# imulki/serenade

Measured on AMD Instinct MI355X. Metric: mel frames/sec converted (UNet ODE + vocoder), 80x1024, higher is better.
Workload: dtype f32

## Files before the change

### include/serenade_hip.h

```cpp
#ifndef SERENADE_HIP_H
#define SERENADE_HIP_H

#include <stdint.h>

#ifdef __cplusplus
extern "C" {
#endif

#define SRN_ABI_VERSION 4
#define SRN_MAX_TAPS 16

enum { SRN_ACT_NONE = 0, SRN_ACT_LEAKY = 1, SRN_ACT_SILU = 2, SRN_ACT_MISH = 3 };
enum { SRN_RES_NONE = 0, SRN_RES_ADD = 1, SRN_RES_AXPY = 2 };
enum {
  SRN_POST_NONE = 0,
  SRN_POST_DIV = 1,
  SRN_POST_TANH = 2,
  SRN_POST_RELU = 3,
  SRN_POST_LEAKY = 4,
  SRN_POST_GELU = 5
};
enum {
  SRN_PREC_FP32 = 0,
  SRN_PREC_BF16X3 = 1,
  SRN_PREC_BF16X6 = 2
};
enum {
  SRN_ROUTE_AUTO = 0,
  SRN_ROUTE_TILED = 1,
  SRN_ROUTE_HALO = 2,
  SRN_ROUTE_GENERIC = 3,
  SRN_ROUTE_STRIP = 4,
  SRN_ROUTE_FAST_FP32 = 5
};
enum {
  SRN_FAMILY_GENERIC = 0,
  SRN_FAMILY_F32 = 1,
  SRN_FAMILY_FAST = 2,
  SRN_FAMILY_HALO = 3,
  SRN_FAMILY_STRIP = 4
};

typedef struct SrnConvParams {
  int32_t n_batch;
  int32_t n_head;
  int32_t T_in, T_out;
  int32_t C_in;
  int32_t C_in0;
  int32_t C_w;
  int32_t N;
  int32_t N_out;
  int32_t n_taps;
  int32_t tap_off[SRN_MAX_TAPS];
  int32_t in_stride;
  int32_t pad_reflect;
  int32_t w_nmajor;
  int32_t pro_act;
  float pro_slope;
  float alpha;
  float beta;
  int32_t geglu;
  int32_t res_mode;
  int32_t post;
  float post_div;
  int32_t out_t_stride, out_t_off;
  int32_t tile;
  const float* in0; int64_t in0_bs, in0_hs; int32_t ld_in0;
  const float* in1; int64_t in1_bs; int32_t ld_in1;
  const float* w;   int64_t w_bs, w_hs; int32_t ldw;
  const float* bias;
  const int32_t* len_in;
  const int32_t* len_out;
  const float* res;  int64_t res_bs, res_hs; int32_t ld_res;
  const float* res2; int64_t res2_bs; int32_t ld_res2;
  float* out; int64_t out_bs, out_hs; int32_t ld_out;
  int32_t precision;
  int32_t route;
  void* ws; int64_t ws_bytes;
  const void* w_hi; const void* w_lo;
  float* gn_partials;
  float* out_tr; int64_t out_tr_bs; int32_t ld_out_tr; int32_t out_tr_col0;
} SrnConvParams;

int srn_abi_version(void);
const char* srn_last_error(void);

int srn_conv_gemm(const SrnConvParams* p, void* stream);
int64_t srn_conv_gemm_workspace_bytes(const SrnConvParams* p);
int srn_conv_gemm_route(const SrnConvParams* p, int32_t out[3]);

int srn_gn_mish_apply(const float* x, const float* gn_partials, const float* gamma, const float* beta,
                      const float* time_bias, int64_t time_bias_bs, const int32_t* lens, float* y, int B, int T,
                      int C, int groups, float eps, int valid_stats, void* stream);

int srn_resblock_tail(const float* c2, const float* gn_partials, const float* gamma, const float* beta,
                      const int32_t* lens, const float* r, const float* scale, const float* shift, int64_t ld_ss,
                      float* y, int B, int T, int C, int groups, float gn_eps, float ln_eps, int valid_stats,
                      void* stream);

int srn_resblock_tail_ln(const float* c2, const float* gn_partials, const float* gamma, const float* beta,
                         const int32_t* lens, const float* r, const float* scale, const float* shift, int64_t ld_ss,
                         float* y, int B, int T, int C, int groups, float gn_eps, float ln_eps, int valid_stats,
                         const float* ln2_gamma, const float* ln2_beta, float* y2, float ln2_eps, void* stream);

int srn_layernorm(const float* x, const float* gamma, const float* beta, float* y, int64_t rows, int C, float eps,
                  void* stream);

int srn_softmax_rows(float* s, const int32_t* lens, int Z, int n_head, int L, int ld, void* stream);

int srn_sinusoidal_emb(const float* t, float* out, int n, int dim, int ld, float scale, void* stream);

int srn_copy_channels(const float* src, int64_t src_bs, int ld_src, int sc0, float* dst, int64_t dst_bs, int ld_dst,
                      int dc0, int B, int T, int C, void* stream);

int srn_scatter_rows(const float* src, int64_t src_bs, int ld_src, float* dst, int64_t dst_bs, int ld_dst, int dc0,
                     const int32_t* row_off, const int32_t* n_rows, int B, int T, int C, void* stream);

int srn_transpose_ct(const float* src, float* dst, int B, int R, int Cc, int64_t src_bs, int ld_src, int64_t dst_bs,
                     int ld_dst, void* stream);
#define SRN_TR_LIST_MAX 40
typedef struct SrnTransposeList {
  int32_t n;
  int32_t pad_;
  const float* src[SRN_TR_LIST_MAX];
  float* dst[SRN_TR_LIST_MAX];
  int64_t src_bs[SRN_TR_LIST_MAX], dst_bs[SRN_TR_LIST_MAX];
  int32_t B[SRN_TR_LIST_MAX], R[SRN_TR_LIST_MAX], Cc[SRN_TR_LIST_MAX];
  int32_t ld_src[SRN_TR_LIST_MAX], ld_dst[SRN_TR_LIST_MAX];
  int32_t first_block[SRN_TR_LIST_MAX + 1];
} SrnTransposeList;
int srn_transpose_multi(const SrnTransposeList* list, void* stream);

int srn_renorm(const float* x, const float* trg_scale, const float* trg_mean, const float* voc_mean,
               const float* voc_scale, float* y, int64_t rows, int C, void* stream);

int srn_out_conv_tanh(const float* x, const float* w, const float* bias, float* y, int B, int T, int C, int k,
                      float slope, void* stream);

typedef struct SrnResUnitParams {
  int32_t n_batch, T, C;
  int32_t k, dilation;
  float slope;
  const float* x; int64_t x_bs;
  const float* w1; const float* b1; const float* w2; const float* b2;
  const void* w1_hi; const void* w2_hi;
  const float* res2; int64_t res2_bs;
  float post_div;
  float* out; int64_t out_bs;
  int32_t precision;
  int32_t route;
} SrnResUnitParams;
enum { SRN_RESUNIT_ROUTE_SHARED = 1 };

int srn_hifigan_resunit(const SrnResUnitParams* p, void* stream);

int srn_pd_gather(const float* x, const float* d, float* out, int B, int T, int C, float dilation, float slope,
                  void* stream);

int srn_gru_recur_last(const float* gi, const float* w_hh_t, const float* b_hh, float* h, int B, int T, int H,
                       void* stream);

int srn_style_token_attention_kv(const float* ref, const float* wq_t, const float* bq, const float* k, const float* v,
                                 const float* wo_t, const float* bo, float* out, int B, int Dq, int n_tok, int F,
                                 int n_head, void* stream);

int srn_pad_signal(const float* x, float* out, int B, int n, int pad, int ld, int mode, void* stream);
int srn_logmel(const float* spec, const float* mel_t, float* out, int64_t frames, int n_bins, int ld, int n_mels,
               float eps, int log_mode, void* stream);
int srn_loudness(const float* spec, const float* a_weight_db, uint32_t* gmax_ws, float* out, int B, int frames,
                 int n_bins, int ld, float amin, float top_db, float add_eps, void* stream);

int srn_rowln_fwd(const float* x, const float* m, int64_t m_bs, const float* a, int64_t a_bs, float* y, int B, int T,
                  int C, float eps, void* stream);
int srn_rowln_bwd(const float* x, const float* dy, const float* m, int64_t m_bs, float* dx, float* partial, int B, int T,
                  int C, float eps, void* stream);
int srn_rowln_chunks(int T);
int srn_gn_mish_bwd_partial(const float* h, const float* dy, const float* mean, const float* rstd, const float* gamma,
                            const float* beta, const int32_t* lens, float* partial, int B, int T, int C, int groups,
                            void* stream);
int srn_gn_mish_bwd_apply(const float* h, const float* dy, const float* mean, const float* rstd, const float* gamma,
                          const float* beta, const float* gsum, const int32_t* lens, float* dh, int B, int T, int C,
                          int groups, void* stream);
int srn_gn_chunks(int T);
int srn_gn_stats(const float* partials, float* mean, float* rstd, int B, int T, int C, int groups, float eps,
                 void* stream);
int srn_chunk_colsum(const float* partial, const float* gamma, float* col, float* gsum, int B, int n_chunk, int C,
                     int groups, void* stream);
int srn_colsum(const float* x, float* partial, float* out, int B, int64_t R, int N, int ld, void* stream);
int srn_colsum_chunks(int64_t R);
int srn_softmax_bwd(const float* p, float* dp, int64_t rows, int L, int ld, float scale, void* stream);
int srn_geglu_fwd(const float* hg, float* a, int64_t rows, int inner, void* stream);
int srn_geglu_bwd(const float* hg, const float* da, float* dhg, int64_t rows, int inner, void* stream);
int srn_adamw(float* p, const float* g, float* m, float* v, int64_t n, float lr, float beta1, float beta2, float eps,
              float weight_decay, int step, float grad_scale, void* stream);
int srn_adamw_dyn(float* p, const float* g, float* m, float* v, int64_t n, float beta1, float beta2, float eps,
                  float weight_decay, const float* dyn, void* stream);
int srn_sumsq(const float* g, int64_t n, double* partial, void* stream);
int srn_dot(const float* a, const float* b, int64_t n, double* partial, void* stream);
#define SRN_COPY_LIST_MAX 160
typedef struct SrnCopyList {
  int32_t n;
  int32_t pad_;
  const void* src[SRN_COPY_LIST_MAX];
  int64_t off[SRN_COPY_LIST_MAX];
  int64_t len[SRN_COPY_LIST_MAX];
} SrnCopyList;
int srn_multi_copy(const SrnCopyList* list, float* dst, void* stream);
int srn_sumsq_blocks(int64_t n);
int srn_weight_norm_fwd(const float* v, const float* g, float* w_packed, float* wd, float* inv_norm, int N, int C, int k,
                        void* stream);
int srn_weight_norm_bwd(const float* dw_packed, const float* v, const float* g, const float* inv_norm, float* dv,
                        float* dg, int N, int C, int k, void* stream);

typedef struct SrnWorldParams {
  int32_t n_batch, max_frames;
  int32_t fs, fft_size;
  const double* x; int64_t x_bs; const int32_t* x_len;
  const double* f0; const double* t; int64_t f_bs;
  const int32_t* n_frames;
  const double* twiddle;
  double q1, f0_floor;
  double threshold;
  double unvoiced_db;
  const double* band_window; int32_t band_window_len;
  int32_t n_bands;
  double* out0; int64_t out0_bs; int32_t ld_out0;
  double* out1; int64_t out1_bs; int32_t ld_out1;
} SrnWorldParams;
int srn_world_cheaptrick(const SrnWorldParams* p, void* stream);
int srn_world_d4c(const SrnWorldParams* p, void* stream);
int srn_world_project(const double* in, int64_t rows, int K, int ld_in, const double* mat_t, int n_out, int take_log,
                      double* out, int ld_out, void* stream);
int srn_world_pack_features(const double* a, int na, const double* b, int nb, const double* mean, const double* scale,
                            float* out, int64_t rows, int ld_out, void* stream);
int srn_wave_to_f64(const float* wave, double* out, int64_t n, int pcm16, void* stream);
int srn_f0_match_length(const double* in, int64_t in_bs, const int32_t* n_in, double* out, int64_t out_bs,
                        const int32_t* n_out, int n_batch, int max_out, void* stream);
int srn_cont_f0(const double* f0, int64_t bs, const int32_t* n_frames, double* cf0, float* uv, int32_t* ok,
                int n_batch, void* stream);
typedef struct SrnExcitationParams {
  int32_t n_batch, max_frames, fs, hop;
  const double* f0;
  const double* df_f0;
  int64_t f_bs;
  const int32_t* n_frames;
  double* phase_ws;
  const float* noise;
  float* sine;
  float sine_amp, noise_amp;
  int32_t n_df;
  float* dfs[4];
  int32_t df_upsample[4];
  double dense_factors[4];
} SrnExcitationParams;
int srn_sifigan_excitation(const SrnExcitationParams* p, void* stream);

typedef struct SrnTnGemmParams {
  int32_t n_batch, n_head;
  int32_t n_items, T_a, T_b;
  int32_t stride, n_shifts;
  int32_t shift[SRN_MAX_TAPS];
  int32_t M, N;
  const float* a; int64_t a_bs, a_hs, a_is; int32_t lda;
  const float* b; int64_t b_bs, b_hs, b_is; int32_t ldb;
  float* out; int64_t out_bs, out_hs; int32_t ldc;
  float alpha;
  float* ws; int64_t ws_bytes;
  int32_t n_inner;
  int64_t a_is2, b_is2;
  const int32_t* len_b;
  float* colsum;
  int32_t route;
} SrnTnGemmParams;
enum { SRN_TN_ROUTE_GENERAL = 1 };
int srn_tn_gemm(const SrnTnGemmParams* p, void* stream);
int64_t srn_tn_gemm_workspace_bytes(const SrnTnGemmParams* p);

int srn_bn_chunks(int64_t rows);
int srn_bn_relu_fwd(const float* x, const float* gamma, const float* beta, float* run_mean, float* run_var,
                    float* partial, float* stats, float* y, int64_t rows, int C, float eps, float momentum, void* stream);
int srn_bn_relu_bwd(const float* x, const float* y, const float* dy, const float* stats, const float* gamma,
                    float* partial, float* sums, float* dx, int64_t rows, int C, void* stream);
int srn_im2col_s2(const float* x, float* col, int B, int H, int W, int C, int ld, void* stream);
int srn_col2im_s2(const float* col, float* dx, int B, int H, int W, int C, int ld, void* stream);
int srn_gru_train_fwd(const float* gi, const float* w_hh_t, const float* b_hh, float* hs, float* gates, int B, int T,
                      int H, void* stream);
int srn_gru_train_bwd(const float* dh_last, const float* w_hh, const float* hs, const float* gates, float* dgi,
                      float* dgh, int B, int T, int H, void* stream);
int srn_token_attn_fwd(const float* q, const float* k, const float* v, float* p, float* ctx, int B, int n_tok, int F,
                       int n_head, void* stream);
int srn_token_attn_bwd(const float* dctx, const float* q, const float* k, const float* v, const float* p, float* dq,
                       float* dk_part, float* dv_part, int B, int n_tok, int F, int n_head, void* stream);

int srn_frame_stats_chunks(int T);
int srn_cvec_conv0(const float* wave, int64_t wave_bs, int n, const int32_t* lens, const float* w, float* out,
                   double* partials, int B, int T0, int C, int k, int stride, void* stream);
int srn_channel_norm_gelu(const float* x, const double* partials, int n_chunks, const int32_t* lens,
                          const float* gamma, const float* beta, float* stats, float* y, int B, int T, int C, float eps,
                          void* stream);
int srn_posconv_gelu_res(const float* x, const int32_t* lens, const float* w, const float* bias, float* y, int B,
                         int T, int C, int groups, int k, int pad, void* stream);

int srn_pad_ragged(const float* x, int64_t x_bs, const int32_t* lens, float* out, int B, int n, int pad, int ld,
                   void* stream);
int srn_mel_db(const float* spec, int ld_spec, int n_bins, const float* mel_t, const int32_t* lens, unsigned* gmax_ws,
               float* out, int ld_out, int B, int T, int n_mels, float amin, float top_db, void* stream);
int srn_trans_conv0(const float* x, int64_t x_bs, int ld_x, const int32_t* lens, const float* w, const float* bias,
                    float* out, int B, int T, int F, int C, int dilation, void* stream);
int srn_trans_pool(const float* in, const int32_t* lens, float* out, int B, int T, int F_in, int C, int C_valid,
                   int flatten, int ld_out, void* stream);
int srn_bilstm_slices(int H);
int srn_bilstm_recur(const float* g, int64_t g_bs, int ld_g, const int32_t* lens, const float* w_hh_t, float* out,
                     int64_t out_bs, int ld_out, int B, int T, int H, void* stream);

#define SRN_PYIN_MAX_FRAME 4096
#define SRN_PYIN_MAX_PERIODS 1024
#define SRN_PYIN_MAX_STATES 4096
#define SRN_PYIN_MAX_THRESHOLDS 1024
int srn_pyin_observe(const float* x, int64_t x_bs, const int32_t* lens, const int32_t* frames, const double* thresholds,
                     const double* beta_probs, const double* boltz_fact, const double* boltz_exp,
                     const double* no_trough, double* obs, double* voiced_prob, int B, int N, int T, int frame_length,
                     int win_length, int hop_length, int pad, int min_period, int max_period, int n_thresholds,
                     double sr, double fmin, double bins_per_octave, int n_bins, void* stream);
int srn_pyin_viterbi(const double* obs, const double* voiced_prob, const int32_t* frames, const double* log_band,
                     const double* log_p_init, const double* freqs, double log_tiny, double fill_na, int fill_unvoiced,
                     uint16_t* ptr_ws, int32_t* states, double* f0, uint8_t* voiced_flag, int B, int T, int n_bins,
                     int width, void* stream);

#ifdef __cplusplus
}
#endif
#endif
```

### serenade_amd/_lib.py

```python
import ctypes
import os
from ctypes import POINTER, c_char_p, c_double, c_float, c_int, c_int32, c_int64, c_void_p

_HERE = os.path.dirname(os.path.abspath(__file__))
LIB_PATH = os.environ.get("SERENADE_AMD_LIB") or os.path.join(_HERE, "libserenade_hip.so")

SRN_MAX_TAPS = 16
ACT_NONE, ACT_LEAKY, ACT_SILU, ACT_MISH = 0, 1, 2, 3
RES_NONE, RES_ADD, RES_AXPY = 0, 1, 2
POST_NONE, POST_DIV, POST_TANH, POST_RELU, POST_LEAKY, POST_GELU = 0, 1, 2, 3, 4, 5
PREC_FP32, PREC_BF16X3, PREC_BF16X6 = 0, 1, 2
ROUTE_AUTO, ROUTE_TILED, ROUTE_HALO, ROUTE_GENERIC, ROUTE_STRIP, ROUTE_FAST_FP32 = 0, 1, 2, 3, 4, 5
FAMILY_GENERIC, FAMILY_F32, FAMILY_FAST, FAMILY_HALO, FAMILY_STRIP = 0, 1, 2, 3, 4
RESUNIT_ROUTE_SHARED = 1
TN_ROUTE_GENERAL = 1


class SrnConvParams(ctypes.Structure):
    _fields_ = [
        ("n_batch", c_int32), ("n_head", c_int32), ("T_in", c_int32), ("T_out", c_int32),
        ("C_in", c_int32), ("C_in0", c_int32), ("C_w", c_int32), ("N", c_int32), ("N_out", c_int32),
        ("n_taps", c_int32), ("tap_off", c_int32 * SRN_MAX_TAPS), ("in_stride", c_int32),
        ("pad_reflect", c_int32), ("w_nmajor", c_int32), ("pro_act", c_int32), ("pro_slope", c_float),
        ("alpha", c_float), ("beta", c_float), ("geglu", c_int32), ("res_mode", c_int32), ("post", c_int32), ("post_div", c_float),
        ("out_t_stride", c_int32), ("out_t_off", c_int32), ("tile", c_int32),
        ("in0", c_void_p), ("in0_bs", c_int64), ("in0_hs", c_int64), ("ld_in0", c_int32),
        ("in1", c_void_p), ("in1_bs", c_int64), ("ld_in1", c_int32),
        ("w", c_void_p), ("w_bs", c_int64), ("w_hs", c_int64), ("ldw", c_int32),
        ("bias", c_void_p), ("len_in", c_void_p), ("len_out", c_void_p),
        ("res", c_void_p), ("res_bs", c_int64), ("res_hs", c_int64), ("ld_res", c_int32),
        ("res2", c_void_p), ("res2_bs", c_int64), ("ld_res2", c_int32),
        ("out", c_void_p), ("out_bs", c_int64), ("out_hs", c_int64), ("ld_out", c_int32),
        ("precision", c_int32), ("route", c_int32), ("ws", c_void_p), ("ws_bytes", c_int64),
        ("w_hi", c_void_p), ("w_lo", c_void_p), ("gn_partials", c_void_p),
        ("out_tr", c_void_p), ("out_tr_bs", c_int64), ("ld_out_tr", c_int32), ("out_tr_col0", c_int32),
    ]


class SrnResUnitParams(ctypes.Structure):
    _fields_ = [
        ("n_batch", c_int32), ("T", c_int32), ("C", c_int32), ("k", c_int32), ("dilation", c_int32),
        ("slope", c_float), ("x", c_void_p), ("x_bs", c_int64),
        ("w1", c_void_p), ("b1", c_void_p), ("w2", c_void_p), ("b2", c_void_p),
        ("w1_hi", c_void_p), ("w2_hi", c_void_p), ("res2", c_void_p), ("res2_bs", c_int64),
        ("post_div", c_float), ("out", c_void_p), ("out_bs", c_int64), ("precision", c_int32), ("route", c_int32),
    ]


SRN_COPY_LIST_MAX = 160


class SrnCopyList(ctypes.Structure):
    _fields_ = [("n", c_int32), ("pad_", c_int32), ("src", c_void_p * SRN_COPY_LIST_MAX),
                ("off", c_int64 * SRN_COPY_LIST_MAX), ("len", c_int64 * SRN_COPY_LIST_MAX)]


class SrnWorldParams(ctypes.Structure):
    _fields_ = [
        ("n_batch", c_int32), ("max_frames", c_int32), ("fs", c_int32), ("fft_size", c_int32),
        ("x", c_void_p), ("x_bs", c_int64), ("x_len", c_void_p),
        ("f0", c_void_p), ("t", c_void_p), ("f_bs", c_int64), ("n_frames", c_void_p), ("twiddle", c_void_p),
        ("q1", c_double), ("f0_floor", c_double), ("threshold", c_double), ("unvoiced_db", c_double),
        ("band_window", c_void_p), ("band_window_len", c_int32), ("n_bands", c_int32),
        ("out0", c_void_p), ("out0_bs", c_int64), ("ld_out0", c_int32),
        ("out1", c_void_p), ("out1_bs", c_int64), ("ld_out1", c_int32),
    ]


SRN_TR_LIST_MAX = 40


class SrnTransposeList(ctypes.Structure):
    _fields_ = [("n", c_int32), ("pad_", c_int32), ("src", c_void_p * SRN_TR_LIST_MAX), ("dst", c_void_p * SRN_TR_LIST_MAX),
                ("src_bs", c_int64 * SRN_TR_LIST_MAX), ("dst_bs", c_int64 * SRN_TR_LIST_MAX),
                ("B", c_int32 * SRN_TR_LIST_MAX), ("R", c_int32 * SRN_TR_LIST_MAX), ("Cc", c_int32 * SRN_TR_LIST_MAX),
                ("ld_src", c_int32 * SRN_TR_LIST_MAX), ("ld_dst", c_int32 * SRN_TR_LIST_MAX),
                ("first_block", c_int32 * (SRN_TR_LIST_MAX + 1))]


class SrnTnGemmParams(ctypes.Structure):
    _fields_ = [
        ("n_batch", c_int32), ("n_head", c_int32), ("n_items", c_int32), ("T_a", c_int32), ("T_b", c_int32),
        ("stride", c_int32), ("n_shifts", c_int32), ("shift", c_int32 * SRN_MAX_TAPS), ("M", c_int32), ("N", c_int32),
        ("a", c_void_p), ("a_bs", c_int64), ("a_hs", c_int64), ("a_is", c_int64), ("lda", c_int32),
        ("b", c_void_p), ("b_bs", c_int64), ("b_hs", c_int64), ("b_is", c_int64), ("ldb", c_int32),
        ("out", c_void_p), ("out_bs", c_int64), ("out_hs", c_int64), ("ldc", c_int32),
        ("alpha", c_float), ("ws", c_void_p), ("ws_bytes", c_int64),
        ("n_inner", c_int32), ("a_is2", c_int64), ("b_is2", c_int64), ("len_b", c_void_p), ("colsum", c_void_p),
        ("route", c_int32),
    ]


class SrnExcitationParams(ctypes.Structure):
    _fields_ = [
        ("n_batch", c_int32), ("max_frames", c_int32), ("fs", c_int32), ("hop", c_int32),
        ("f0", c_void_p), ("df_f0", c_void_p), ("f_bs", c_int64), ("n_frames", c_void_p), ("phase_ws", c_void_p),
        ("noise", c_void_p), ("sine", c_void_p), ("sine_amp", c_float), ("noise_amp", c_float), ("n_df", c_int32),
        ("dfs", c_void_p * 4), ("df_upsample", c_int32 * 4), ("dense_factors", c_double * 4),
    ]


_P = c_void_p
_SIGS = {
    "srn_abi_version": (c_int, []),
    "srn_last_error": (c_char_p, []),
    "srn_conv_gemm": (c_int, [POINTER(SrnConvParams), _P]),
    "srn_conv_gemm_workspace_bytes": (c_int64, [POINTER(SrnConvParams)]),
    "srn_conv_gemm_route": (c_int, [POINTER(SrnConvParams), POINTER(c_int32)]),
    "srn_hifigan_resunit": (c_int, [POINTER(SrnResUnitParams), _P]),
    "srn_gn_mish_apply": (c_int, [_P, _P, _P, _P, _P, c_int64, _P, _P, c_int, c_int, c_int, c_int, c_float, c_int, _P]),
    "srn_resblock_tail": (c_int, [_P, _P, _P, _P, _P, _P, _P, _P, c_int64, _P, c_int, c_int, c_int, c_int,
                                  c_float, c_float, c_int, _P]),
    "srn_resblock_tail_ln": (c_int, [_P, _P, _P, _P, _P, _P, _P, _P, c_int64, _P, c_int, c_int, c_int, c_int,
                                     c_float, c_float, c_int, _P, _P, _P, c_float, _P]),
    "srn_scatter_rows": (c_int, [_P, c_int64, c_int, _P, c_int64, c_int, c_int, _P, _P, c_int, c_int, c_int, _P]),
    "srn_layernorm": (c_int, [_P, _P, _P, _P, c_int64, c_int, c_float, _P]),
    "srn_softmax_rows": (c_int, [_P, _P, c_int, c_int, c_int, c_int, _P]),
    "srn_sinusoidal_emb": (c_int, [_P, _P, c_int, c_int, c_int, c_float, _P]),
    "srn_copy_channels": (c_int, [_P, c_int64, c_int, c_int, _P, c_int64, c_int, c_int, c_int, c_int, c_int, _P]),
    "srn_transpose_ct": (c_int, [_P, _P, c_int, c_int, c_int, c_int64, c_int, c_int64, c_int, _P]),
    "srn_transpose_multi": (c_int, [POINTER(SrnTransposeList), _P]),
    "srn_weight_norm_fwd": (c_int, [_P, _P, _P, _P, _P, c_int, c_int, c_int, _P]),
    "srn_weight_norm_bwd": (c_int, [_P, _P, _P, _P, _P, _P, c_int, c_int, c_int, _P]),
    "srn_renorm": (c_int, [_P, _P, _P, _P, _P, _P, c_int64, c_int, _P]),
    "srn_out_conv_tanh": (c_int, [_P, _P, _P, _P, c_int, c_int, c_int, c_int, c_float, _P]),
    "srn_pd_gather": (c_int, [_P, _P, _P, c_int, c_int, c_int, c_float, c_float, _P]),
    "srn_pad_signal": (c_int, [_P, _P, c_int, c_int, c_int, c_int, c_int, _P]),
    "srn_logmel": (c_int, [_P, _P, _P, c_int64, c_int, c_int, c_int, c_float, c_int, _P]),
    "srn_loudness": (c_int, [_P, _P, _P, _P, c_int, c_int, c_int, c_int, c_float, c_float, c_float, _P]),
    "srn_gru_recur_last": (c_int, [_P, _P, _P, _P, c_int, c_int, c_int, _P]),
    "srn_style_token_attention_kv": (c_int, [_P] * 8 + [c_int] * 5 + [_P]),
    "srn_rowln_fwd": (c_int, [_P, _P, c_int64, _P, c_int64, _P, c_int, c_int, c_int, c_float, _P]),
    "srn_rowln_bwd": (c_int, [_P, _P, _P, c_int64, _P, _P, c_int, c_int, c_int, c_float, _P]),
    "srn_rowln_chunks": (c_int, [c_int]),
    "srn_gn_mish_bwd_partial": (c_int, [_P] * 8 + [c_int] * 4 + [_P]),
    "srn_gn_mish_bwd_apply": (c_int, [_P] * 9 + [c_int] * 4 + [_P]),
    "srn_gn_chunks": (c_int, [c_int]),
    "srn_gn_stats": (c_int, [_P, _P, _P, c_int, c_int, c_int, c_int, c_float, _P]),
    "srn_chunk_colsum": (c_int, [_P, _P, _P, _P, c_int, c_int, c_int, c_int, _P]),
    "srn_colsum": (c_int, [_P, _P, _P, c_int, c_int64, c_int, c_int, _P]),
    "srn_colsum_chunks": (c_int, [c_int64]),
    "srn_softmax_bwd": (c_int, [_P, _P, c_int64, c_int, c_int, c_float, _P]),
    "srn_geglu_fwd": (c_int, [_P, _P, c_int64, c_int, _P]),
    "srn_geglu_bwd": (c_int, [_P, _P, _P, c_int64, c_int, _P]),
    "srn_adamw": (c_int, [_P, _P, _P, _P, c_int64, c_float, c_float, c_float, c_float, c_float, c_int, c_float, _P]),
    "srn_adamw_dyn": (c_int, [_P, _P, _P, _P, c_int64, c_float, c_float, c_float, c_float, _P, _P]),
    "srn_sumsq": (c_int, [_P, c_int64, _P, _P]),
    "srn_dot": (c_int, [_P, _P, c_int64, _P, _P]),
    "srn_multi_copy": (c_int, [POINTER(SrnCopyList), _P, _P]),
    "srn_sumsq_blocks": (c_int, [c_int64]),
    "srn_bn_chunks": (c_int, [c_int64]),
    "srn_bn_relu_fwd": (c_int, [_P] * 8 + [c_int64, c_int, c_float, c_float, _P]),
    "srn_bn_relu_bwd": (c_int, [_P] * 8 + [c_int64, c_int, _P]),
    "srn_im2col_s2": (c_int, [_P, _P] + [c_int] * 5 + [_P]),
    "srn_col2im_s2": (c_int, [_P, _P] + [c_int] * 5 + [_P]),
    "srn_gru_train_fwd": (c_int, [_P] * 5 + [c_int] * 3 + [_P]),
    "srn_gru_train_bwd": (c_int, [_P] * 6 + [c_int] * 3 + [_P]),
    "srn_token_attn_fwd": (c_int, [_P] * 5 + [c_int] * 4 + [_P]),
    "srn_token_attn_bwd": (c_int, [_P] * 8 + [c_int] * 4 + [_P]),
    "srn_tn_gemm": (c_int, [POINTER(SrnTnGemmParams), _P]),
    "srn_tn_gemm_workspace_bytes": (c_int64, [POINTER(SrnTnGemmParams)]),
    "srn_world_cheaptrick": (c_int, [POINTER(SrnWorldParams), _P]),
    "srn_world_d4c": (c_int, [POINTER(SrnWorldParams), _P]),
    "srn_world_project": (c_int, [_P, c_int64, c_int, c_int, _P, c_int, c_int, _P, c_int, _P]),
    "srn_world_pack_features": (c_int, [_P, c_int, _P, c_int, _P, _P, _P, c_int64, c_int, _P]),
    "srn_wave_to_f64": (c_int, [_P, _P, c_int64, c_int, _P]),
    "srn_f0_match_length": (c_int, [_P, c_int64, _P, _P, c_int64, _P, c_int, c_int, _P]),
    "srn_cont_f0": (c_int, [_P, c_int64, _P, _P, _P, _P, c_int, _P]),
    "srn_sifigan_excitation": (c_int, [POINTER(SrnExcitationParams), _P]),
    "srn_frame_stats_chunks": (c_int, [c_int]),
    "srn_cvec_conv0": (c_int, [_P, c_int64, c_int, _P, _P, _P, _P] + [c_int] * 5 + [_P]),
    "srn_channel_norm_gelu": (c_int, [_P, _P, c_int, _P, _P, _P, _P, _P, c_int, c_int, c_int, c_float, _P]),
    "srn_posconv_gelu_res": (c_int, [_P] * 5 + [c_int] * 6 + [_P]),
    "srn_pad_ragged": (c_int, [_P, c_int64, _P, _P, c_int, c_int, c_int, c_int, _P]),
    "srn_mel_db": (c_int, [_P, c_int, c_int, _P, _P, _P, _P, c_int, c_int, c_int, c_int, c_float, c_float, _P]),
    "srn_trans_conv0": (c_int, [_P, c_int64, c_int, _P, _P, _P, _P] + [c_int] * 5 + [_P]),
    "srn_trans_pool": (c_int, [_P, _P, _P] + [c_int] * 7 + [_P]),
    "srn_bilstm_slices": (c_int, [c_int]),
    "srn_bilstm_recur": (c_int, [_P, c_int64, c_int, _P, _P, _P, c_int64, c_int, c_int, c_int, c_int, _P]),
    "srn_pyin_observe": (c_int, [_P, c_int64] + [_P] * 9 + [c_int] * 10 + [c_double] * 3 + [c_int, _P]),
    "srn_pyin_viterbi": (c_int, [_P] * 6 + [c_double] * 2 + [c_int] + [_P] * 4 + [c_int] * 4 + [_P]),
}

EXPORTS = tuple(_SIGS)

_lib = None


def lib():
    global _lib
    if _lib is None:
        if not os.path.exists(LIB_PATH):
            raise RuntimeError(
                f"{LIB_PATH} not found: build it with `python -m serenade_amd.build` "
                "(hipcc --offload-arch=gfx950). There is no CPU fallback.")
        h = ctypes.CDLL(LIB_PATH)
        for name, (res, args) in _SIGS.items():
            fn = getattr(h, name)
            fn.restype = res
            fn.argtypes = args
        if h.srn_abi_version() != 4:
            raise RuntimeError("libserenade_hip.so ABI version mismatch")
        _lib = h
    return _lib


def check(rc, what=""):
    if rc != 0:
        msg = lib().srn_last_error().decode("utf-8", "replace")
        raise RuntimeError(f"libserenade_hip {what} failed (rc={rc}): {msg}")
```

### serenade_amd/csrc/resunit_f32.hip

```cpp
#include <hip/hip_runtime.h>

#include "common.h"
#include "conv_common.h"
#include "serenade_hip.h"

namespace {

constexpr int HALO_MAX = 50;
constexpr int NTH = 512;

typedef unsigned u32x4r __attribute__((ext_vector_type(4)));

struct FDivR {
  uint32_t mul, shift;
};
__device__ __forceinline__ int fdivr(const int n, const FDivR d) {
  return (int)(((uint64_t)(uint32_t)n * d.mul) >> d.shift);
}

template <int C_>
struct UCfg {
  static constexpr int C = C_, CH = C / 32;
  static constexpr int BMI = C == 32 ? 256 : 128;
  static constexpr int A_ROWS = BMI + HALO_MAX + 2;
  static constexpr int A_PLANE = A_ROWS * 144;
  static constexpr int A_BYTES = CH * A_PLANE;
  static constexpr int UNIT = C * 144;
  static constexpr int G = 9216 / UNIT >= 2 ? 2 : 1;
  static constexpr int STAGE = G * UNIT;
  static constexpr int SMEM = A_BYTES + 2 * STAGE;
  static constexpr int F4R = C / 4, RSTEP = NTH / F4R;
  static constexpr int A_LD = (A_ROWS * F4R + NTH - 1) / NTH;
  static_assert(G * C * 8 == NTH, "one 16-B weight piece per thread per stage");
};

template <class R>
__global__ __launch_bounds__(NTH, 4) void resunit_f32_kernel(const SrnResUnitParams p, const int tiles_per_z,
                                                             const int n_tiles, const FDivR d_tpz) {
  constexpr int C = R::C, CH = R::CH, BMI = R::BMI, G = R::G;
  extern __shared__ __attribute__((aligned(16))) unsigned char smem_u[];
  unsigned char* const sA = smem_u;
  unsigned char* const sW = smem_u + R::A_BYTES;

  const int tid = threadIdx.x;
  const int lane = tid & 63;
  const int wave = __builtin_amdgcn_readfirstlane(tid >> 6);
  const int li = lane & 31;
  const int lh = lane >> 5;
  const int k = p.k, dil = p.dilation, T = p.T;
  const int p2 = (k - 1) / 2, p1 = p2 * dil;
  const int BMo = BMI - (k - 1);
  const int hr = BMI + (k - 1) * dil;
  const int U = k * CH;
  const int S = (U + G - 1) / G;
  const float slope = p.slope;

  const int w_n = (tid % (C * 8)) >> 3;
  const int w_g = tid / (C * 8);
  const int w_voff = w_n * (k * C * 4) + w_g * 128 + (tid & 7) * 16;
  const int w_dst = (w_g * C + w_n) * 144 + (tid & 7) * 16;
  const int w_bytes = C * k * C * 4;
  const __amdgpu_buffer_rsrc_t rs_w1 = __builtin_amdgcn_make_buffer_rsrc(const_cast<float*>(p.w1), 0, w_bytes, 0x00020000);
  const __amdgpu_buffer_rsrc_t rs_w2 = __builtin_amdgcn_make_buffer_rsrc(const_cast<float*>(p.w2), 0, w_bytes, 0x00020000);
  u32x4r wr;
  auto w_load = [&](const int j) {
    if (j >= S) wr = __builtin_amdgcn_raw_buffer_load_b128(rs_w2, w_voff, (j - S) * G * 128, 0);
    else wr = __builtin_amdgcn_raw_buffer_load_b128(rs_w1, w_voff, j * G * 128, 0);
  };
  auto w_store = [&](const int buf) {
    *reinterpret_cast<u32x4r*>(sW + buf * R::STAGE + w_dst) = wr;
  };

  constexpr int A_LD = R::A_LD, F4R = R::F4R, RSTEP = R::RSTEP;
  const int a_f4 = tid % F4R;
  const int a_r0 = tid / F4R;
  const int a_voff = (a_r0 * C + a_f4 * 4) * 4;
  const int a_dst0 = (a_f4 >> 3) * R::A_PLANE + a_r0 * 144 + (a_f4 & 7) * 16;
  u32x4r pa[A_LD];
  auto load_a = [&](const int tile) {
    const int z = fdivr(tile, d_tpz);
    const int t0 = (tile - z * tiles_per_z) * BMo;
    const __amdgpu_buffer_rsrc_t rs_x =
        __builtin_amdgcn_make_buffer_rsrc(const_cast<float*>(p.x + (int64_t)z * p.x_bs), 0, T * C * 4, 0x00020000);
    const int v0 = a_voff + (t0 - p2 - p1) * (C * 4);
#pragma unroll
    for (int j = 0; j < A_LD; ++j) pa[j] = __builtin_amdgcn_raw_buffer_load_b128(rs_x, v0 + j * (RSTEP * C * 4), 0, 0);
  };
  auto stage_a = [&]() {
#pragma unroll
    for (int j = 0; j < A_LD; ++j) {
      if (a_r0 + RSTEP * j < hr) {
        float4 v = __builtin_bit_cast(float4, pa[j]);
        v.x = fmaxf(v.x, v.x * slope);
        v.y = fmaxf(v.y, v.y * slope);
        v.z = fmaxf(v.z, v.z * slope);
        v.w = fmaxf(v.w, v.w * slope);
        *reinterpret_cast<float4*>(sA + a_dst0 + j * RSTEP * 144) = v;
      }
    }
  };

  const int wm0 = (C == 64 ? (wave & 3) : wave) * 32;
  const int ng0 = C == 64 ? (wave >> 2) : 0;
  const int fa_lane = (wm0 + li) * 144 + 16 * lh;
  const int fb_lane = R::A_BYTES + (ng0 * 32 + li) * 144 + 16 * lh;
  f32x16 acc;
  auto zero_acc = [&]() {
#pragma unroll
    for (int r = 0; r < 16; ++r) acc[r] = 0.f;
  };

  auto compute = [&](const int buf, const int u0, const int step) {
#pragma unroll
    for (int g = 0; g < G; ++g) {
      const int u = u0 + g;
      if (u >= U) break;
      const int tap = u / CH;
      const int c = u - tap * CH;
      const float* a = reinterpret_cast<const float*>(smem_u + (fa_lane + (c * R::A_PLANE + tap * step * 144)));
      const float* b = reinterpret_cast<const float*>(smem_u + (fb_lane + (buf * R::STAGE + g * C * 144)));
#pragma unroll
      for (int kk = 0; kk < 4; ++kk) {
        const float4 af = *reinterpret_cast<const float4*>(a + kk * 8);
        const float4 bf = *reinterpret_cast<const float4*>(b + kk * 8);
        acc = __builtin_amdgcn_mfma_f32_32x32x2f32(af.x, bf.x, acc, 0, 0, 0);
        acc = __builtin_amdgcn_mfma_f32_32x32x2f32(af.y, bf.y, acc, 0, 0, 0);
        acc = __builtin_amdgcn_mfma_f32_32x32x2f32(af.z, bf.z, acc, 0, 0, 0);
        acc = __builtin_amdgcn_mfma_f32_32x32x2f32(af.w, bf.w, acc, 0, 0, 0);
      }
    }
  };

  int wj = 0, wbuf = 0;
  auto conv_pass = [&](const int step) {
    for (int s = 0; s < S; ++s) {
      compute(wbuf, s * G, step);
      w_store(wbuf ^ 1);
      int nxt = wj + 2;
      if (nxt >= 2 * S) nxt -= 2 * S;
      w_load(nxt);
      wj = wj + 1 == 2 * S ? 0 : wj + 1;
      wbuf ^= 1;
      __syncthreads();
    }
  };

  int tile = blockIdx.x;
  load_a(tile);
  w_load(0);
  w_store(0);
  w_load(2 * S > 1 ? 1 : 0);

  const float bias1 = p.b1[ng0 * 32 + li];
  const float bias2 = p.b2[ng0 * 32 + li];
  const bool divide = p.post_div != 0.f && p.post_div != 1.f;
  const bool has_q = p.res2 != nullptr;
  const int mid_lane = ng0 * R::A_PLANE + ((wm0 + 4 * lh) * 36 + li) * 4;
  const int io_lane = ((wm0 + 4 * lh) * C + ng0 * 32 + li) * 4;

  for (; tile < n_tiles; tile += gridDim.x) {
    const int z = fdivr(tile, d_tpz);
    const int t0 = (tile - z * tiles_per_z) * BMo;
    stage_a();
    __syncthreads();
    const int next = tile + gridDim.x;
    load_a(next < n_tiles ? next : tile);

    zero_acc();
    conv_pass(dil);
    if (t0 - p2 >= 0 && t0 - p2 + BMI <= T) {
#pragma unroll
      for (int r = 0; r < 16; ++r) {
        const float v = acc[r] + bias1;
        *reinterpret_cast<float*>(sA + mid_lane + ((r & 3) + 8 * (r >> 2)) * 144) = fmaxf(v, v * slope);
      }
    } else {
#pragma unroll
      for (int r = 0; r < 16; ++r) {
        const int dr = (r & 3) + 8 * (r >> 2);
        const int gi = t0 - p2 + wm0 + 4 * lh + dr;
        float v = acc[r] + bias1;
        v = fmaxf(v, v * slope);
        if (gi < 0 || gi >= T) v = 0.f;
        *reinterpret_cast<float*>(sA + mid_lane + dr * 144) = v;
      }
    }
    __syncthreads();

    zero_acc();
    conv_pass(1);

    const int row_end = min(BMo, T - t0);
    const int64_t zoff = (int64_t)t0 * C;
    const int io_bytes = row_end * C * 4;
    const __amdgpu_buffer_rsrc_t rs_xe = __builtin_amdgcn_make_buffer_rsrc(
        const_cast<float*>(p.x + (int64_t)z * p.x_bs + zoff), 0, io_bytes, 0x00020000);
    const __amdgpu_buffer_rsrc_t rs_qe = __builtin_amdgcn_make_buffer_rsrc(
        const_cast<float*>(has_q ? p.res2 + (int64_t)z * p.res2_bs + zoff : p.x), 0, has_q ? io_bytes : 0, 0x00020000);
    const __amdgpu_buffer_rsrc_t rs_oe =
        __builtin_amdgcn_make_buffer_rsrc(p.out + (int64_t)z * p.out_bs + zoff, 0, io_bytes, 0x00020000);
    if (wm0 + 32 <= row_end) {
#pragma unroll
      for (int gq = 0; gq < 4; ++gq) {
        float xv[4], qv[4];
#pragma unroll
        for (int i = 0; i < 4; ++i) {
          xv[i] = __builtin_bit_cast(float, __builtin_amdgcn_raw_buffer_load_b32(rs_xe, io_lane, (8 * gq + i) * C * 4, 0));
          qv[i] = __builtin_bit_cast(float, __builtin_amdgcn_raw_buffer_load_b32(rs_qe, io_lane, (8 * gq + i) * C * 4, 0));
        }
#pragma unroll
        for (int i = 0; i < 4; ++i) {
          float v = acc[4 * gq + i] + bias2 + xv[i];
          if (has_q) v += qv[i];
          if (divide) v = v / p.post_div;
          __builtin_amdgcn_raw_buffer_store_b32(__builtin_bit_cast(unsigned, v), rs_oe, io_lane, (8 * gq + i) * C * 4, 0);
        }
      }
    } else if (wm0 < row_end) {
#pragma unroll
      for (int gq = 0; gq < 4; ++gq) {
        float xv[4], qv[4];
#pragma unroll
        for (int i = 0; i < 4; ++i) {
          xv[i] = __builtin_bit_cast(float, __builtin_amdgcn_raw_buffer_load_b32(rs_xe, io_lane + (8 * gq + i) * C * 4, 0, 0));
          qv[i] = __builtin_bit_cast(float, __builtin_amdgcn_raw_buffer_load_b32(rs_qe, io_lane + (8 * gq + i) * C * 4, 0, 0));
        }
#pragma unroll
        for (int i = 0; i < 4; ++i) {
          float v = acc[4 * gq + i] + bias2 + xv[i];
          if (has_q) v += qv[i];
          if (divide) v = v / p.post_div;
          __builtin_amdgcn_raw_buffer_store_b32(__builtin_bit_cast(unsigned, v), rs_oe, io_lane + (8 * gq + i) * C * 4, 0, 0);
        }
      }
    }
  }
}

FDivR make_fdivr(const uint32_t d) {
  int lg = 0;
  while ((1u << lg) < d) ++lg;
  const int k = 26 + lg;
  return FDivR{(uint32_t)(((1ull << k) + d - 1) / d), (uint32_t)k};
}

template <class R>
int launch_unit(const SrnResUnitParams& p, hipStream_t stream) {
  static SrnSmemAttr smem_attr;
  if (const int e = smem_attr.ensure(reinterpret_cast<const void*>(&resunit_f32_kernel<R>), R::SMEM)) return e;
  const int BMo = R::BMI - (p.k - 1);
  const int tiles_per_z = (p.T + BMo - 1) / BMo;
  const int64_t n_tiles = (int64_t)p.n_batch * tiles_per_z;
  if (n_tiles <= 0 || n_tiles >= (1ll << 26)) return 0;
  const int grid = (int)(n_tiles < 512 ? n_tiles : 512);
  hipLaunchKernelGGL((resunit_f32_kernel<R>), dim3(grid), dim3(NTH), R::SMEM, stream, p, tiles_per_z, (int)n_tiles,
                     make_fdivr((uint32_t)tiles_per_z));
  SRN_CHECK_LAUNCH();
  return 1;
}

}

int srn_resunit_f32_try(const SrnResUnitParams& p, hipStream_t stream) {
  if (!(p.slope >= 0.f && p.slope <= 1.f)) return 0;
  if ((int64_t)p.T * p.C * 4 >= 0x7fffffffll) return 0;
  return p.C == 32 ? launch_unit<UCfg<32>>(p, stream) : launch_unit<UCfg<64>>(p, stream);
}
```

Before: 61510.

## Assign contiguous tile spans per block and carry conv1 halo rows between tiles

Each block now processes a contiguous span of time tiles within one batch item instead of a strided set of overlapping tiles. The last k-1 rows of the first conv output are carried in registers into the next tile's LDS, so later tiles yield BMI output rows instead of BMI-(k-1) and skip recomputing the overlap. Residual and skip input loads for the epilogue are also issued before the first conv pass to hide their latency. The cost is more indexing logic, extra registers for the carry and the early-loaded values, and possible load imbalance from the fixed span grid.

```diff
diff --git a/include/serenade_hip.h b/include/serenade_hip.h
--- a/include/serenade_hip.h
+++ b/include/serenade_hip.h
@@ -150,7 +150,7 @@
   int32_t precision;
   int32_t route;
 } SrnResUnitParams;
-enum { SRN_RESUNIT_ROUTE_SHARED = 1 };
+enum { SRN_RESUNIT_ROUTE_SHARED = 1, SRN_RESUNIT_ROUTE_OVERLAPPED = 2 };
 
 int srn_hifigan_resunit(const SrnResUnitParams* p, void* stream);
 
diff --git a/serenade_amd/_lib.py b/serenade_amd/_lib.py
--- a/serenade_amd/_lib.py
+++ b/serenade_amd/_lib.py
@@ -13,6 +13,7 @@
 ROUTE_AUTO, ROUTE_TILED, ROUTE_HALO, ROUTE_GENERIC, ROUTE_STRIP, ROUTE_FAST_FP32 = 0, 1, 2, 3, 4, 5
 FAMILY_GENERIC, FAMILY_F32, FAMILY_FAST, FAMILY_HALO, FAMILY_STRIP = 0, 1, 2, 3, 4
 RESUNIT_ROUTE_SHARED = 1
+RESUNIT_ROUTE_OVERLAPPED = 2
 TN_ROUTE_GENERAL = 1
 
 
diff --git a/serenade_amd/csrc/resunit_f32.hip b/serenade_amd/csrc/resunit_f32.hip
--- a/serenade_amd/csrc/resunit_f32.hip
+++ b/serenade_amd/csrc/resunit_f32.hip
@@ -8,6 +8,10 @@
 
 constexpr int HALO_MAX = 50;
 constexpr int NTH = 512;
+
+#ifndef SRN_RESUNIT_EPI_EARLY
+#define SRN_RESUNIT_EPI_EARLY 1
+#endif
 
 typedef unsigned u32x4r __attribute__((ext_vector_type(4)));
 
@@ -17,6 +21,11 @@
 __device__ __forceinline__ int fdivr(const int n, const FDivR d) {
   return (int)(((uint64_t)(uint32_t)n * d.mul) >> d.shift);
 }
+
+struct SpanPlan {
+  int spz, q, r;
+  FDivR d_spz;
+};
 
 template <int C_>
 struct UCfg {
@@ -36,7 +45,7 @@
 
 template <class R>
 __global__ __launch_bounds__(NTH, 4) void resunit_f32_kernel(const SrnResUnitParams p, const int tiles_per_z,
-                                                             const int n_tiles, const FDivR d_tpz) {
+                                                             const int n_tiles, const FDivR d_tpz, const SpanPlan sp) {
   constexpr int C = R::C, CH = R::CH, BMI = R::BMI, G = R::G;
   extern __shared__ __attribute__((aligned(16))) unsigned char smem_u[];
   unsigned char* const sA = smem_u;
@@ -77,12 +86,33 @@
   const int a_voff = (a_r0 * C + a_f4 * 4) * 4;
   const int a_dst0 = (a_f4 >> 3) * R::A_PLANE + a_r0 * 144 + (a_f4 & 7) * 16;
   u32x4r pa[A_LD];
-  auto load_a = [&](const int tile) {
-    const int z = fdivr(tile, d_tpz);
-    const int t0 = (tile - z * tiles_per_z) * BMo;
+  const bool sliding = sp.spz != 0;
+  int span_z = 0, span_t0 = 0, n_my;
+  if (sliding) {
+    span_z = fdivr(blockIdx.x, sp.d_spz);
+    const int s = blockIdx.x - span_z * sp.spz;
+    n_my = sp.q + (s < sp.r ? 1 : 0);
+    span_t0 = (s * sp.q + min(s, sp.r)) * BMI - s * (k - 1);
+  } else {
+    n_my = (n_tiles - (int)blockIdx.x + (int)gridDim.x - 1) / (int)gridDim.x;
+  }
+  auto tile_pos = [&](const int it, int& z, int& t0) {
+    if (sliding) {
+      z = span_z;
+      t0 = span_t0 + it * BMI - (it ? k - 1 : 0);
+    } else {
+      const int tile = blockIdx.x + it * gridDim.x;
+      z = fdivr(tile, d_tpz);
+      t0 = (tile - z * tiles_per_z) * BMo;
+    }
+  };
+  auto load_a = [&](const int it) {
+    int z, t0;
+    tile_pos(it, z, t0);
+    const int m0 = sliding && it ? t0 + p2 : t0 - p2;
     const __amdgpu_buffer_rsrc_t rs_x =
         __builtin_amdgcn_make_buffer_rsrc(const_cast<float*>(p.x + (int64_t)z * p.x_bs), 0, T * C * 4, 0x00020000);
-    const int v0 = a_voff + (t0 - p2 - p1) * (C * 4);
+    const int v0 = a_voff + (m0 - p1) * (C * 4);
 #pragma unroll
     for (int j = 0; j < A_LD; ++j) pa[j] = __builtin_amdgcn_raw_buffer_load_b128(rs_x, v0 + j * (RSTEP * C * 4), 0, 0);
   };
@@ -145,8 +175,7 @@
     }
   };
 
-  int tile = blockIdx.x;
-  load_a(tile);
+  load_a(0);
   w_load(0);
   w_store(0);
   w_load(2 * S > 1 ? 1 : 0);
@@ -158,39 +187,27 @@
   const int mid_lane = ng0 * R::A_PLANE + ((wm0 + 4 * lh) * 36 + li) * 4;
   const int io_lane = ((wm0 + 4 * lh) * C + ng0 * 32 + li) * 4;
 
-  for (; tile < n_tiles; tile += gridDim.x) {
-    const int z = fdivr(tile, d_tpz);
-    const int t0 = (tile - z * tiles_per_z) * BMo;
+  const int n_carry = (k - 1) * C;
+  float carry[2] = {0.f, 0.f};
+  int carry_lds[2];
+#pragma unroll
+  for (int i = 0; i < 2; ++i) {
+    const int e = tid + NTH * i, col = e % C;
+    carry_lds[i] = (col >> 5) * R::A_PLANE + (e / C) * 144 + (col & 31) * 4;
+  }
+
+  for (int it = 0; it < n_my; ++it) {
+    int z, t0;
+    tile_pos(it, z, t0);
+    const bool first = !sliding || it == 0;
+    const int m0 = first ? t0 - p2 : t0 + p2;
+    const int mrow = first ? 0 : k - 1;
     stage_a();
     __syncthreads();
-    const int next = tile + gridDim.x;
-    load_a(next < n_tiles ? next : tile);
-
-    zero_acc();
-    conv_pass(dil);
-    if (t0 - p2 >= 0 && t0 - p2 + BMI <= T) {
-#pragma unroll
-      for (int r = 0; r < 16; ++r) {
-        const float v = acc[r] + bias1;
-        *reinterpret_cast<float*>(sA + mid_lane + ((r & 3) + 8 * (r >> 2)) * 144) = fmaxf(v, v * slope);
-      }
-    } else {
-#pragma unroll
-      for (int r = 0; r < 16; ++r) {
-        const int dr = (r & 3) + 8 * (r >> 2);
-        const int gi = t0 - p2 + wm0 + 4 * lh + dr;
-        float v = acc[r] + bias1;
-        v = fmaxf(v, v * slope);
-        if (gi < 0 || gi >= T) v = 0.f;
-        *reinterpret_cast<float*>(sA + mid_lane + dr * 144) = v;
-      }
-    }
-    __syncthreads();
-
-    zero_acc();
-    conv_pass(1);
-
-    const int row_end = min(BMo, T - t0);
+    load_a(it + 1 < n_my ? it + 1 : it);
+
+    const int rows_out = first ? BMo : BMI;
+    const int row_end = max(min(rows_out, T - t0), 0);
     const int64_t zoff = (int64_t)t0 * C;
     const int io_bytes = row_end * C * 4;
     const __amdgpu_buffer_rsrc_t rs_xe = __builtin_amdgcn_make_buffer_rsrc(
@@ -199,39 +216,87 @@
         const_cast<float*>(has_q ? p.res2 + (int64_t)z * p.res2_bs + zoff : p.x), 0, has_q ? io_bytes : 0, 0x00020000);
     const __amdgpu_buffer_rsrc_t rs_oe =
         __builtin_amdgcn_make_buffer_rsrc(p.out + (int64_t)z * p.out_bs + zoff, 0, io_bytes, 0x00020000);
-    if (wm0 + 32 <= row_end) {
-#pragma unroll
-      for (int gq = 0; gq < 4; ++gq) {
-        float xv[4], qv[4];
-#pragma unroll
-        for (int i = 0; i < 4; ++i) {
-          xv[i] = __builtin_bit_cast(float, __builtin_amdgcn_raw_buffer_load_b32(rs_xe, io_lane, (8 * gq + i) * C * 4, 0));
-          qv[i] = __builtin_bit_cast(float, __builtin_amdgcn_raw_buffer_load_b32(rs_qe, io_lane, (8 * gq + i) * C * 4, 0));
-        }
-#pragma unroll
-        for (int i = 0; i < 4; ++i) {
-          float v = acc[4 * gq + i] + bias2 + xv[i];
-          if (has_q) v += qv[i];
-          if (divide) v = v / p.post_div;
-          __builtin_amdgcn_raw_buffer_store_b32(__builtin_bit_cast(unsigned, v), rs_oe, io_lane, (8 * gq + i) * C * 4, 0);
-        }
+    const bool whole = wm0 + 32 <= row_end;
+    float xv[16], qv[16];
+#if SRN_RESUNIT_EPI_EARLY
+    if (whole) {
+#pragma unroll
+      for (int r = 0; r < 16; ++r) {
+        xv[r] = __builtin_bit_cast(float, __builtin_amdgcn_raw_buffer_load_b32(rs_xe, io_lane, ((r & 3) + 8 * (r >> 2)) * C * 4, 0));
+        qv[r] = __builtin_bit_cast(float, __builtin_amdgcn_raw_buffer_load_b32(rs_qe, io_lane, ((r & 3) + 8 * (r >> 2)) * C * 4, 0));
+      }
+    } else {
+#pragma unroll
+      for (int r = 0; r < 16; ++r) {
+        xv[r] = __builtin_bit_cast(float, __builtin_amdgcn_raw_buffer_load_b32(rs_xe, io_lane + ((r & 3) + 8 * (r >> 2)) * C * 4, 0, 0));
+        qv[r] = __builtin_bit_cast(float, __builtin_amdgcn_raw_buffer_load_b32(rs_qe, io_lane + ((r & 3) + 8 * (r >> 2)) * C * 4, 0, 0));
+      }
+    }
+#endif
+
+    zero_acc();
+    conv_pass(dil);
+    if (m0 >= 0 && m0 + BMI <= T) {
+#pragma unroll
+      for (int r = 0; r < 16; ++r) {
+        const float v = acc[r] + bias1;
+        *reinterpret_cast<float*>(sA + mid_lane + (mrow + (r & 3) + 8 * (r >> 2)) * 144) = fmaxf(v, v * slope);
+      }
+    } else {
+#pragma unroll
+      for (int r = 0; r < 16; ++r) {
+        const int dr = (r & 3) + 8 * (r >> 2);
+        const int gi = m0 + wm0 + 4 * lh + dr;
+        float v = acc[r] + bias1;
+        v = fmaxf(v, v * slope);
+        if (gi < 0 || gi >= T) v = 0.f;
+        *reinterpret_cast<float*>(sA + mid_lane + (mrow + dr) * 144) = v;
+      }
+    }
+    if (!first) {
+#pragma unroll
+      for (int i = 0; i < 2; ++i)
+        if (tid + NTH * i < n_carry) *reinterpret_cast<float*>(sA + carry_lds[i]) = carry[i];
+    }
+    __syncthreads();
+    if (sliding) {
+#pragma unroll
+      for (int i = 0; i < 2; ++i)
+        if (tid + NTH * i < n_carry) carry[i] = *reinterpret_cast<const float*>(sA + carry_lds[i] + (mrow + BMo) * 144);
+    }
+
+    zero_acc();
+    conv_pass(1);
+
+    if (whole) {
+#if !SRN_RESUNIT_EPI_EARLY
+#pragma unroll
+      for (int r = 0; r < 16; ++r) {
+        xv[r] = __builtin_bit_cast(float, __builtin_amdgcn_raw_buffer_load_b32(rs_xe, io_lane, ((r & 3) + 8 * (r >> 2)) * C * 4, 0));
+        qv[r] = __builtin_bit_cast(float, __builtin_amdgcn_raw_buffer_load_b32(rs_qe, io_lane, ((r & 3) + 8 * (r >> 2)) * C * 4, 0));
+      }
+#endif
+#pragma unroll
+      for (int r = 0; r < 16; ++r) {
+        float v = acc[r] + bias2 + xv[r];
+        if (has_q) v += qv[r];
+        if (divide) v = v / p.post_div;
+        __builtin_amdgcn_raw_buffer_store_b32(__builtin_bit_cast(unsigned, v), rs_oe, io_lane, ((r & 3) + 8 * (r >> 2)) * C * 4, 0);
       }
     } else if (wm0 < row_end) {
-#pragma unroll
-      for (int gq = 0; gq < 4; ++gq) {
-        float xv[4], qv[4];
-#pragma unroll
-        for (int i = 0; i < 4; ++i) {
-          xv[i] = __builtin_bit_cast(float, __builtin_amdgcn_raw_buffer_load_b32(rs_xe, io_lane + (8 * gq + i) * C * 4, 0, 0));
-          qv[i] = __builtin_bit_cast(float, __builtin_amdgcn_raw_buffer_load_b32(rs_qe, io_lane + (8 * gq + i) * C * 4, 0, 0));
-        }
-#pragma unroll
-        for (int i = 0; i < 4; ++i) {
-          float v = acc[4 * gq + i] + bias2 + xv[i];
-          if (has_q) v += qv[i];
-          if (divide) v = v / p.post_div;
-          __builtin_amdgcn_raw_buffer_store_b32(__builtin_bit_cast(unsigned, v), rs_oe, io_lane + (8 * gq + i) * C * 4, 0, 0);
-        }
+#if !SRN_RESUNIT_EPI_EARLY
+#pragma unroll
+      for (int r = 0; r < 16; ++r) {
+        xv[r] = __builtin_bit_cast(float, __builtin_amdgcn_raw_buffer_load_b32(rs_xe, io_lane + ((r & 3) + 8 * (r >> 2)) * C * 4, 0, 0));
+        qv[r] = __builtin_bit_cast(float, __builtin_amdgcn_raw_buffer_load_b32(rs_qe, io_lane + ((r & 3) + 8 * (r >> 2)) * C * 4, 0, 0));
+      }
+#endif
+#pragma unroll
+      for (int r = 0; r < 16; ++r) {
+        float v = acc[r] + bias2 + xv[r];
+        if (has_q) v += qv[r];
+        if (divide) v = v / p.post_div;
+        __builtin_amdgcn_raw_buffer_store_b32(__builtin_bit_cast(unsigned, v), rs_oe, io_lane + ((r & 3) + 8 * (r >> 2)) * C * 4, 0, 0);
       }
     }
   }
@@ -242,6 +307,19 @@
   while ((1u << lg) < d) ++lg;
   const int k = 26 + lg;
   return FDivR{(uint32_t)(((1ull << k) + d - 1) / d), (uint32_t)k};
+}
+
+SpanPlan plan_spans(const int n_batch, const int T, const int k, const int BMI) {
+  SpanPlan sp{0, 0, 0, {0, 0}};
+  const int spz = 512 / n_batch;
+  if (spz < 1 || n_batch * spz < 480) return sp;
+  const int64_t nt = ((int64_t)T + (int64_t)spz * (k - 1) + BMI - 1) / BMI;
+  if (nt < 2 * spz) return sp;
+  sp.spz = spz;
+  sp.q = (int)(nt / spz);
+  sp.r = (int)(nt % spz);
+  sp.d_spz = make_fdivr((uint32_t)spz);
+  return sp;
 }
 
 template <class R>
@@ -252,9 +330,11 @@
   const int tiles_per_z = (p.T + BMo - 1) / BMo;
   const int64_t n_tiles = (int64_t)p.n_batch * tiles_per_z;
   if (n_tiles <= 0 || n_tiles >= (1ll << 26)) return 0;
-  const int grid = (int)(n_tiles < 512 ? n_tiles : 512);
+  SpanPlan sp{0, 0, 0, {0, 0}};
+  if (p.route != SRN_RESUNIT_ROUTE_OVERLAPPED) sp = plan_spans(p.n_batch, p.T, p.k, R::BMI);
+  const int grid = sp.spz ? p.n_batch * sp.spz : (int)(n_tiles < 512 ? n_tiles : 512);
   hipLaunchKernelGGL((resunit_f32_kernel<R>), dim3(grid), dim3(NTH), R::SMEM, stream, p, tiles_per_z, (int)n_tiles,
-                     make_fdivr((uint32_t)tiles_per_z));
+                     make_fdivr((uint32_t)tiles_per_z), sp);
   SRN_CHECK_LAUNCH();
   return 1;
 }
```

New measurement: 61670, median of 6. No clear change (+0.3%).
